# nikhilTkur/Multigrid_dolfinx

Hardware: AMD Instinct MI355X
Metric: V-cycles/sec + achieved HBM GB/s, 3D Poisson P1 1024³ DoF, 1/2/4/8 MI355X (higher is better)
Workload: dtype f64

## Files before the change

### include/mg_hip.h

```cpp
#ifndef MG_HIP_H
#define MG_HIP_H

#include <stddef.h>
#include <stdint.h>

#ifdef __cplusplus
extern "C" {
#endif

typedef struct mg_context* mg_handle;

enum mg_vec {
    MG_VEC_V = 0,
    MG_VEC_F = 1,
    MG_VEC_R = 2,
    MG_VEC_ERR = 3
};

enum mg_restriction {
    MG_RESTRICT_INJECTION = 0,
    MG_RESTRICT_FULL_WEIGHTING = 1,
    MG_RESTRICT_TABLE = 2,
    MG_RESTRICT_P1_TRANSPOSE = 3
};
// ... 142 lines not shown
    MG_PATH_SWEEP1C = 1,
    MG_PATH_PAIR_CLASS = 2,
    MG_PATH_PAIR_PLAIN = 3,
    MG_PATH_KSWEEP = 4,
    MG_PATH_KSWEEP_ESCAPE = 5,
    MG_PATH_KSWEEP_SLAB = 6,
    MG_PATH_BLOCK = 7,
    MG_PATH_K2D = 8,
    MG_PATH_SMALL = 9,
    MG_PATH_MATRIX_FREE = 10,
    MG_PATH_COUNT = 11
};
int mg_smoother_launches(mg_handle h, int level, int path, int64_t* launches, int64_t* sweeps, int64_t* tail_launches);
int mg_reset_smoother_launches(mg_handle h);

int mg_time_kernel(mg_handle h, const char* kernel, int level, int reps, double* avg_ms);
int mg_sync(mg_handle h);
int mg_memory_bytes(mg_handle h, int64_t* bytes);

#ifdef __cplusplus
}
#endif
#endif
```

### multigrid_dolfinx_amd/_capi.py

```python
from __future__ import annotations

import ctypes as C
import os

import numpy as np

_HERE = os.path.dirname(os.path.abspath(__file__))
LIB_PATH = os.path.join(_HERE, "libmg_hip.so")

MG_VEC_V, MG_VEC_F, MG_VEC_R, MG_VEC_ERR = 0, 1, 2, 3
MG_RESTRICT_INJECTION, MG_RESTRICT_FULL_WEIGHTING, MG_RESTRICT_TABLE, MG_RESTRICT_P1_TRANSPOSE = 0, 1, 2, 3
MG_SMOOTH_JACOBI, MG_SMOOTH_RBGS, MG_SMOOTH_MCGS, MG_SMOOTH_CHEBYSHEV = 0, 1, 2, 3
MG_NORM_L2, MG_NORM_MASS = 0, 1
MG_KAPPA_ARITHMETIC, MG_KAPPA_HARMONIC = 0, 1
MG_NODES_INTERIOR, MG_NODES_ALL = 0, 1
MG_BATCH_MAX = 32
MG_BATCH_JACOBI, MG_BATCH_RESIDUAL, MG_BATCH_SPMV = 0, 1, 2
SMOOTHER_PATHS = ("slice", "sweep1c", "pair_class", "pair_plain", "ksweep", "ksweep_escape", "ksweep_slab", "block", "k2d",
                  "small", "matrix_free")

EXCHANGE_FN = C.CFUNCTYPE(C.c_int, C.c_void_p, C.POINTER(C.c_double), C.POINTER(C.c_double),
                          C.POINTER(C.c_double), C.POINTER(C.c_double), C.c_int64)
ALLREDUCE_FN = C.CFUNCTYPE(C.c_int, C.c_void_p, C.POINTER(C.c_double), C.c_int64)
ALLGATHERV_FN = C.CFUNCTYPE(C.c_int, C.c_void_p, C.POINTER(C.c_double), C.c_int64,
# ... 81 lines not shown
    "mg_prepare_cycle": [_H, C.c_int],
    "mg_norm2": [_H, C.c_int, C.c_int, _dp],
    "mg_quadratic_form": [_H, C.c_int, C.c_int, _dp],
    "mg_set_rhs_true": [_H, C.c_int, C.c_void_p],
    "mg_fmg": [_H, C.c_int, C.c_int, C.c_double, C.c_int, C.c_void_p, _ip],
    "mg_set_mass_csr": [_H, C.c_int, C.c_int64, C.c_int64, C.c_void_p, C.c_int, C.c_void_p, C.c_void_p],
    "mg_set_exact": [_H, C.c_int, C.c_void_p],
    "mg_fmg_ex": [_H, C.c_int, C.c_int, C.c_double, C.c_int, C.c_int, C.c_void_p, C.c_void_p, _ip],
    "mg_pcg": [_H, C.c_int, C.c_double, C.c_int, C.c_void_p, _ip],
    "mg_apply_batch": [_H, C.c_int, C.c_int, C.c_int, C.c_void_p, C.c_void_p, C.c_void_p, C.c_void_p],
    "mg_pcg_batch": [_H, C.c_int, C.c_int, C.c_void_p, C.c_void_p, C.c_double, C.c_int, C.c_void_p, C.c_void_p],
    "mg_batch_info": [_H, _ip, _i64p],
    "mg_release_batch": [_H],
    "mg_counters": [_H, _i64p, _i64p, _i64p, _ip],
    "mg_smoother_launches": [_H, C.c_int, C.c_int, _i64p, _i64p, _i64p],
    "mg_reset_smoother_launches": [_H],
    "mg_time_kernel": [_H, C.c_char_p, C.c_int, C.c_int, _dp],
    "mg_sync": [_H],
    "mg_memory_bytes": [_H, _i64p],
}

_lib = None


class MgError(RuntimeError):
    """A non-zero status from libmg_hip.so; the message is mg_last_error()."""


def build_extension():
    import subprocess
# ... 37 lines not shown
```

### multigrid_dolfinx_amd/csrc/mg_capi.hip

```cpp
#include "../../include/mg_hip.h"
#include "mg_csr_check.h"
#include "mg_kernels.hip.h"
#include "mg_direct.hip.h"
#include "mg_jacobi2.hip.h"
#include "mg_jacobik3d.hip.h"
#include "mg_jacobiblk.hip.h"
#include "mg_lattice.hip.h"
#include "mg_diffusion_mf.hip.h"
#include "mg_diffusion_mf_batch.hip.h"
#include "mg_diffusion_adj.hip.h"
#include "mg_diffusion_flux.hip.h"
#include "mg_diffusion_kappa.hip.h"

#include <dlfcn.h>
#include <rccl/rccl.h>

#include <algorithm>
#include <array>
#include <cmath>
#include <cstdio>
#include <cstdlib>
#include <cstring>
#include <initializer_list>
#include <memory>
// ... 134 lines not shown
    bool sdia = false;
    int wu = 0;
    int up[8] = {0, 0, 0, 0, 0, 0, 0, 0};
    int64_t mlead = 0, mslices = 0;
    DevBuf<unsigned char> cls;
    DevBuf<double> ctab;
    int ncls = 0;
    DevBuf<unsigned char> scls;
    DevBuf<int> s_off;
    DevBuf<double> s_val;
    DevBuf<int> s_cnt;
    int nscls = 0;
    DevBuf<int> s_pack;
    int lm_ntop = 0;
    int lm_top[LM_K] = {0, 0, 0, 0, 0, 0, 0, 0};
    int cmain = 0;
    double cm[8] = {0, 0, 0, 0, 0, 0, 0, 0};
    int64_t cls_lead = 0;
    DevBuf<double> dinv;
    bool mf = false;
    DevBuf<double> kappa;
    int faces = MG_FACES_ALL;
    bool diffusion_hierarchy = false;
    bool react = false;
    DevBuf<double> rdiag;
    int robin = 0;
    DVector v, v2, f, err, ftrue;
    DVector sw;
    DVector fcg_x, fcg_p, fcg_q, fcg_b;
    bool cheb_est_ok = false;
// ... 114 lines not shown
    int fuse_k_shape = -1;
    int fuse_k_segments = 0;
    int timing_force_form = -1;
    int64_t fuse_k_slab_min_rows = (int64_t)1 << 20;
    int fuse_k_slab_min_sweeps = 4;
    int64_t fuse_k_min_rows = (int64_t)1 << 24;
    int64_t fuse_k_small_rows = (int64_t)1 << 22;
    int64_t fuse_k5_min_rows = (int64_t)1 << 26;
    int64_t fuse_k4_min_rows = 0;
    int fuse_k_nt_store = 0;
    int fuse_k_min_side = 32;
    int fuse_k_tail = 1;
    int fuse_k_small_tiles = 0;
    int fuse_k_pf = 1;
    int fuse_k_dpp = 1;
    std::vector<const void*> large_lds_kernels;
    int fuse_shape = 1;
    int fuse_wi = 0;
    int fuse_even = 0;
    int march_sweeps = 1;
    int64_t march_min_rows = (int64_t)1 << 22;
    int march_shape = 0;
    int64_t fuse_small_2d_rows = 2048;
    int fuse_small = 1;
    int fuse_2d = 1;
    int fuse_2d_k = 5;
    int fuse_xcd_chunk = 32;
    int cls_blocks_per_cu = 4;
    DirectSolver direct;
    DevTemp ptab_count;
// ... 1217 lines not shown
    MG_TRY(escape_window_k<5>(c, L, cls, clead, &most));
    if (most <= (unsigned)jk3_pool(5)) { *kmax = 5; return 0; }
    MG_TRY(escape_window_k<4>(c, L, cls, clead, &most));
    if (most <= (unsigned)jk3_pool(4)) { *kmax = 4; return 0; }
    MG_TRY(escape_window_k<3>(c, L, cls, clead, &most));
    if (most <= (unsigned)jk3_pool(3)) *kmax = 3;
    return 0;
}

struct JK3Range { int za0, za1, zb0, zb1; };

int jk3_shape(const mg_context* c, int K) {
    return c->fuse_k_shape >= 0 ? c->fuse_k_shape : (K >= 5 ? 8 : 7);
}

template <int K, int NW, int LPW, int M, bool DPP, int PF = 1, int WPE = (NW == 12 ? 3 : 2), int TR = 256, bool ESC = false, bool B1 = false>
int launch_jacobikc_t(mg_context* c, JK3Args a, bool finest, const JK3Range& zr, int seglen) {
    constexpr int EX = 64 * M, EY = NW * LPW, WI = EX - 2 * K, HY = EY - 2 * K + 2;
    a.ntx = (a.nx + WI - 1) / WI;
    a.nty = (a.ny + HY - 1) / HY;
    const int64_t ntile = (int64_t)a.ntx * a.nty;
    constexpr size_t lds = B1 ? jk3b_lds_bytes<K, NW, LPW, M, TR>() : jk3_lds_bytes<K, NW, LPW, M, TR, ESC>();
    static_assert(lds <= 160 * 1024, "one CU's LDS");
    a.za0 = zr.za0; a.za1 = zr.za1; a.zb0 = zr.zb0; a.zb1 = zr.zb1;
    const int planes = std::max(0, zr.za1 - zr.za0) + std::max(0, zr.zb1 - zr.zb0);
    if (planes <= 0) return 0;
    a.ta = (int)ntile; a.seglen_b = 1;
    int64_t items = 0;
    if (seglen <= 0) {
        int64_t cus = std::max(1, c->prop.multiProcessorCount) * (int64_t)std::max<size_t>(1, std::min<size_t>(160 * 1024 / lds, (size_t)(4 * WPE / NW)));
// ... 30 lines not shown
    if (a.ncls > TR) return fail("more row classes than this tile shape keeps in LDS");
    void (*kern)(JK3Args) = nullptr;
    if constexpr (ESC) kern = sdia_jacobikc_escape<K, NW, LPW, M, DPP, PF, WPE, TR>;
    else if constexpr (B1) kern = finest ? sdia_jacobikc_finest_b1<K, NW, LPW, M, WPE, TR> : sdia_jacobikc_b1<K, NW, LPW, M, WPE, TR>;
    else kern = finest ? sdia_jacobikc_finest<K, NW, LPW, M, DPP, PF, WPE, TR> : sdia_jacobikc<K, NW, LPW, M, DPP, PF, WPE, TR>;
    MG_TRY(allow_large_lds(c, reinterpret_cast<const void*>(kern), lds));
    hipLaunchKernelGGL(kern, dim3(grid), dim3(NW * WAVE), lds, c->stream, a);
    HIP_TRY(hipGetLastError());
    c->jk3_tail = a.ta < ntile ? 1 : 0;
    return 0;
}

template <int K, int PF>
int launch_jacobikc_kp(mg_context* c, const JK3Args& a, bool finest, const JK3Range& zr, int seglen) {
    if (!c->fuse_k_dpp) return launch_jacobikc_t<K, 12, 2, 2, false, PF>(c, a, finest, zr, seglen);
    int shape = jk3_shape(c, K) >= 3 && a.ncls > 64 ? 1 : jk3_shape(c, K);
    if (shape == 1 && a.ncls <= 64 && K <= 4 && c->fuse_k_small_tiles) {
        constexpr int WI = 64 - 2 * K, HY = 48 - 2 * K + 2;
        if ((int64_t)((a.nx + WI - 1) / WI) * ((a.ny + HY - 1) / HY) < std::max(1, c->prop.multiProcessorCount)) shape = 4;
    }
    switch (shape) {
        case 1: return launch_jacobikc_t<K, 12, 4, 1, true, PF>(c, a, finest, zr, seglen);
        case 2: return launch_jacobikc_t<K, 8, 3, 2, true, PF>(c, a, finest, zr, seglen);
        case 3: return launch_jacobikc_t<K, 6, 4, 1, true, PF, 3, 64>(c, a, finest, zr, seglen);
        case 4: return launch_jacobikc_t<K, 8, 3, 1, true, PF, 4, 64>(c, a, finest, zr, seglen);
        case 5: if constexpr (K <= 4) return launch_jacobikc_t<K, 4, 6, 1, true, PF, 2, 64>(c, a, finest, zr, seglen);
        case 6: if constexpr (K <= 4 && PF == 1) return launch_jacobikc_t<K, 16, 3, 1, true, 1, 4>(c, a, finest, zr, seglen);
        case 7: return launch_jacobikc_t<K, 16, 2, 1, true, PF, 4>(c, a, finest, zr, seglen);
        case 8: if constexpr (PF == 1) return launch_jacobikc_t<K, 16, 2, 1, true, 1, 4, 256, false, true>(c, a, finest, zr, seglen);
                else return fail("tile shape 8 stages one plane of x (fuse_k_pf 1)");
        default: return launch_jacobikc_t<K, 12, 2, 2, true, PF>(c, a, finest, zr, seglen);
// ... 1 lines not shown
}

template <int K>
int launch_jacobikc_k(mg_context* c, const JK3Args& a, bool finest, const JK3Range& zr, int seglen) {
    if (a.escape) {
        if constexpr (K >= 3) return launch_jacobikc_t<K, 16, 2, 1, true, 1, 4, 256, true>(c, a, finest, zr, seglen);
        else return fail("levels with escape rows take three to five sweeps per pass");
    }
    if constexpr (K == 3 || K == 4) {
        if (c->fuse_k_pf == 2 && (K == 3 || jk3_shape(c, K) == 7)) return launch_jacobikc_kp<K, 2>(c, a, finest, zr, seglen);
    }
    if constexpr (K == 2) return launch_jacobikc_t<K, 12, 4, 1, true, 1>(c, a, finest, zr, seglen);
    else return launch_jacobikc_kp<K, 1>(c, a, finest, zr, seglen);
}

int launch_jacobikc(mg_context* c, const Level& L, int K, const double* x_rows, const double* f_rows, double* out_rows,
                    const JK3Range* zr = nullptr, int seglen = 0) {
    JK3Args a{};
    a.x = x_rows; a.f = f_rows; a.out = out_rows;
    fill_classes_lead(a, L);
    a.P = L.g.plane; a.nx = L.g.nx; a.ny = L.g.ny; a.nz = L.g.nk; a.omega = c->omega;
    const bool dist = is_slab(c, L);
    a.plo = dist && c->comm.rank > 0 ? K : 0;
    a.phi = dist && c->comm.rank + 1 < c->comm.world ? K : 0;
    if (dist && (L.hd < K || L.cls_halo != 1)) return fail("the level's halos are not prepared for that many sweeps per pass");
    if (L.cls_escape && K > L.esc_kmax) return fail("too many escape rows per tile for that many sweeps per pass");
    a.force_form = c->timing_force_form;
    a.nt_store = c->fuse_k_nt_store;
    a.escape = L.cls_escape ? 1 : 0; a.dvals = L.dvals; a.mlead = L.mlead; a.sshift = L.R == 1 ? 6 : (L.R == 2 ? 7 : 8);
    const JK3Range whole{0, L.g.nk, 0, 0};
    c->jk3_tail = 0;
    int rc = 0;
    if (!with_int<2, 3, 4, 5>(K, [&](auto k) { rc = launch_jacobikc_k<decltype(k)::value>(c, a, is_finest(c, L), zr ? *zr : whole, seglen); }))
        return fail("sweeps per pass must be in 2..5");
    return rc;
}

int check_coloring(mg_context* c, Level& L) {
    MG_TRY(need_stored_rows(c, L, "the colouring check of the Gauss-Seidel smoothers"));
    EllArgs a{};
    a.vals = L.vals; a.cols = L.cols; a.codes = L.codes; a.offsets = L.offsets; a.W = L.W;
    a.nloc = L.nloc; a.lead = L.g.lead; a.dinv = L.dinv; a.color_kind = COLOR_LATTICE9; a.grow0 = L.row0; a.gnx = L.g.nx; a.gny = L.g.ny;
    int* d_flag = reinterpret_cast<int*>(c->partials.get());
// ... 1169 lines not shown
                return fail("level " + std::to_string(l) + " is a matrix-free diffusion level: Gauss-Seidel smoothers (RBGS, MCGS) "
                            "need stored rows; use Jacobi or Chebyshev");
    if (!c->direct.tried) { MG_TRY(build_direct(c)); MG_TRY(validate_direct(c)); }
    if (c->smoother == MG_SMOOTH_MCGS)
        for (int l = 1; l <= level; ++l)
            if (c->L[l].mc_ok < 0 && !c->L[l].flat) MG_TRY(check_coloring(c, c->L[l]));
    if (c->comm.active())
        for (int l = 1; l <= level; ++l)
            if (!c->L[l].replicated) {
                MG_TRY(vec_alloc(c, c->L[l], &c->L[l].sw));
                if (c->L[l].cls_halo == 0 && slab_ksweep_level(c, c->L[l]) && std::max(c->mu1, c->mu2) >= c->fuse_k_slab_min_sweeps)
                    MG_TRY(ensure_class_halos(c, c->L[l]));
            }
    if (c->keep_err)
        for (int l = 1; l <= level; ++l) MG_TRY(vec_alloc(c, c->L[l], &c->L[l].err));
    if (c->smoother == MG_SMOOTH_CHEBYSHEV)
        for (int l = 1; l <= level; ++l) {
            double lo = 0.0, hi = 0.0;
            MG_TRY(cheb_interval(c, l, &lo, &hi));
        }
    if (c->p1_prolong || c->restriction == MG_RESTRICT_P1_TRANSPOSE)
        for (int l = 0; l <= level; ++l) MG_TRY(check_p1_stencil(c, c->L[l]));
    return 0;
}

int vcycle_graphed(mg_context* c, int level) {
    MG_TRY(prepare_cycle(c, level));
    const bool slabs = c->comm.active();
    if (!c->use_graph || level == 0 || !c->direct.ok || (slabs && !(c->graph_comm && c->comm.nccl))) return vcycle(c, level);
    std::vector<double*> pre(level + 1);
// ... 626 lines not shown
            return 0;
        }();
        escape = !rc && (double)hist[CLS_ESCAPE] <= 0.25 * (double)L.nloc;
        int kmax = 0;
        if (escape && hist[CLS_ESCAPE] > 0) {
            rc = escape_kmax(c, L, cls, cls_lead, &kmax);
            escape = !rc && kmax >= 3;
        }
        if (std::getenv("MG_DEBUG_STORAGE"))
            std::fprintf(stderr, "[mg] row dictionary with escape: %lld rows, tolerance %d bits, %u escape rows, sweeps per pass that fit %d, rc %d\n",
                         (long long)L.nloc, qbits, hist[CLS_ESCAPE], kmax, rc);
        if (escape) { h[0] = 254; h[1] = 0; L.esc_kmax = kmax; L.rep_escape = hist[CLS_ESCAPE]; }
    }
    if (rc || h[0] > 255 || h[1]) return rc;
    L.cls = std::move(cls); L.ctab = std::move(ctab); L.ncls = h[0] + 1; L.cls_lead = cls_lead;
    L.cls_escape = escape && L.rep_escape > 0;
    if (escape) hist[CLS_ESCAPE] = 0;
    L.cmain = 0;
    for (int k = 1; k < L.ncls; ++k)
        if (L.cmain == 0 || hist[k] > hist[L.cmain]) L.cmain = k;
    for (int t = 0; t < 8; ++t) L.cm[t] = tab[(size_t)CLS_W * L.cmain + t];
    if (L.wu == 4 && !L.cls_escape && !L.flat && L.up[1] == 1 && L.up[2] == L.g.nx && (int64_t)L.up[3] == L.g.plane) {
        JBCheckArgs k{};
        k.cls = L.cls + L.cls_lead; k.ctab = L.ctab; k.nx = L.g.nx; k.ny = L.g.ny; k.nz = L.g.nk; k.P = L.g.plane; k.n = L.nloc;
        k.flag = reinterpret_cast<int*>(c->partials.get());
        HIP_TRY(hipMemsetAsync(k.flag, 0, sizeof(int), c->stream));
        hipLaunchKernelGGL(sdia_grid_decoupled, dim3(blocks_for(L.nloc, 256)), dim3(256), 0, c->stream, k);
        HIP_TRY(hipGetLastError());
        int flag = 1;
        HIP_TRY(hipMemcpyAsync(&flag, k.flag, sizeof(int), hipMemcpyDeviceToHost, c->stream));
// ... 683 lines not shown
    } else if (k == "fuse_k_nt_store") {
        c->fuse_k_nt_store = value != 0;
    } else if (k == "fuse_k_min_side") {
        if (value < 16 || value > 32) return fail("fuse_k_min_side must be in 16..32");
        c->fuse_k_min_side = (int)value;
    } else if (k == "fuse_k_tail") {
        if (value < 0) return fail("fuse_k_tail must be >= 0");
        c->fuse_k_tail = (int)value;
    } else if (k == "fuse_k_small_tiles") {
        c->fuse_k_small_tiles = value != 0;
    } else if (k == "fuse_k_pf") {
        if (value != 1 && value != 2) return fail("fuse_k_pf must be 1 or 2");
        c->fuse_k_pf = (int)value;
    } else if (k == "fuse_k_dpp") {
        c->fuse_k_dpp = value != 0;
    } else if (k == "fuse_k_segments") {
        if (value < 0) return fail("fuse_k_segments must be >= 0");
        c->fuse_k_segments = (int)value;
    } else if (k == "fuse_classes") {
        c->fuse_classes = value != 0;
    } else if (k == "fuse_nontemporal") {
        c->fuse_nontemporal = value != 0;
    } else if (k == "fuse_segments") {
        if (value < 0) return fail("fuse_segments must be >= 0");
        c->fuse_segments = (int)value;
    } else if (k == "coarse_direct") {
        c->use_direct = value != 0;
        free_direct(c);
    } else if (k == "pcg_chunk") {
        if (value < 1) return fail("pcg_chunk must be positive");
// ... 1368 lines not shown
    if (!c) return fail("null handle");
    if (uploads) *uploads = c->uploads;
    if (downloads) *downloads = c->downloads;
    if (graph_replays) *graph_replays = c->graph_replays;
    if (graphs_cached) *graphs_cached = (int)c->graphs.size();
    return 0;
}

int mg_smoother_launches(mg_handle c, int level, int path, int64_t* launches, int64_t* sweeps, int64_t* tail_launches) {
    MG_TRY(check_level(c, level, false));
    if (path < 0 || path >= MG_PATH_COUNT) return fail("smoother path " + std::to_string(path) + " out of range");
    const auto& n = c->smoother_counts[(size_t)level][(size_t)path];
    if (launches) *launches = n.launches;
    if (sweeps) *sweeps = n.sweeps;
    if (tail_launches) *tail_launches = n.tail;
    return 0;
}

int mg_reset_smoother_launches(mg_handle c) {
    if (!c) return fail("null handle");
    for (auto& level : c->smoother_counts) level.fill({});
    return 0;
}

int mg_prepare_cycle(mg_handle c, int level) {
    MG_TRY(check_level(c, level));
    for (int l = 0; l <= level; ++l) {
        MG_TRY(need_matrix(c, l));
        if (level > 0) MG_TRY(need_grid(c, l));
    }
// ... 403 lines not shown
```

### multigrid_dolfinx_amd/csrc/mg_jacobik3d.hip.h

```cpp
#pragma once
#include "mg_jacobi2.hip.h"
#include <type_traits>

namespace mgk {

struct JK3Args {
    const double* x;
    const double* f;
    double* out;
    const unsigned char* cls;
    const double* ctab;
    int64_t clead, P;
    int ncls, cmain;
    double cm[8];
    double omega;
    int nx, ny, nz;
    int plo, phi;
    int ntx, nty, seglen, za0, za1, zb0, zb1;
    int ta, seglen_b;
    unsigned nitems, xcd_chunk;
    int nt_store;
    int escape;
    const double* dvals;
    int64_t mlead;
    int sshift;
    int force_form;
};

constexpr int jk3_pool(int K) { return K >= 5 ? 512 : 1024; }

template <int K, int NW, int LPW, int M, int TR> constexpr size_t jk3_lds_doubles() {
    return TR * CLS_W + (size_t)K * (NW * LPW + 2) * (64 * M) + 2 * (64 * M + 2);
}
template <int K, int NW, int LPW, int M, int TR> constexpr size_t jk3b_lds_doubles() {
    return TR * CLS_W + (size_t)(2 * (K - 1) * (NW * LPW + 1) + 1) * (64 * M);
}
template <int K, int NW, int LPW, int M, int TR> constexpr size_t jk3b_lds_bytes() {
    return sizeof(double) * jk3b_lds_doubles<K, NW, LPW, M, TR>();
}

template <int K, int NW, int LPW, int M, int TR, bool ESC = false> constexpr size_t jk3_lds_bytes() {
    constexpr size_t base = jk3_lds_doubles<K, NW, LPW, M, TR>();
// ... 133 lines not shown
        fn(caps_all{});
    };
    auto cap_of = [&](int c) -> int {
        if constexpr (!CAPS) return K;
        const int ey = ey0 + c / M;
        int cap = min(min(ey + 1, EY - ey), K);
        asm volatile("" : "+v"(cap));
        return __builtin_amdgcn_readfirstlane(cap);
    };

    const int bias = 2 * a.nx + K + 2;
    const int xcl = a.nx + 1 - tx0;
    unsigned eo[NC], eor[M];
#pragma unroll
    for (int c = 0; c < NC; ++c)
        eo[c] = 8u * (unsigned)(min(max(ty0 + ey0 + c / M, -2), a.ny + 1) * a.nx + tx0 + min(lane + 64 * (c % M), xcl) + bias);
#pragma unroll
    for (int r = 0; r < M; ++r)
        eor[r] = 8u * (unsigned)((wlo ? max(ty0 - 1, -2) : min(ty0 + EY, a.ny + 1)) * a.nx + tx0 + min(lane + 64 * r, xcl) + bias);
    unsigned eos[B1 ? M : 1], eon[B1 ? M : 1];
    if constexpr (B1) {
#pragma unroll
        for (int r = 0; r < M; ++r) {
            eos[r] = 8u * (unsigned)(min(max(ty0 + ey0 - 1, -2), a.ny + 1) * a.nx + tx0 + min(lane + 64 * r, xcl) + bias);
            eon[r] = 8u * (unsigned)(min(max(ty0 + ey0 + LPW, -2), a.ny + 1) * a.nx + tx0 + min(lane + 64 * r, xcl) + bias);
        }
    }
    const unsigned char* const clsb = a.cls + a.clead - bias;
    const double* const xb0 = a.x - bias;
    const double* const fb0 = a.f - bias;
    auto sbase = [](const void* p) -> gcptr_t {
        const unsigned long long u = (unsigned long long)p;
        const unsigned lo = (unsigned)__builtin_amdgcn_readfirstlane((int)(unsigned)u);
        const unsigned hi = (unsigned)__builtin_amdgcn_readfirstlane((int)(unsigned)(u >> 32));
        return (gcptr_t)(((unsigned long long)hi << 32) | lo);
    };
    auto ldd = [](gcptr_t b, unsigned e8) -> double {
        asm volatile("" : "+v"(e8));
        return *(const __attribute__((address_space(1))) double*)(b + e8);
    };
    typedef unsigned int __attribute__((aligned(1))) u32_unaligned_t;
    auto ldc = [](gcptr_t b, unsigned e8) -> int {
        unsigned e = e8 >> 3;
        asm volatile("" : "+v"(e));
        return (int)*(const __attribute__((address_space(1))) u32_unaligned_t*)(b + e);
    };
    const int pmin = -a.plo - 1, pmax = a.nz + a.phi;

    double acc[K][NC], fr[K][NC];
    double XA[NC], XB[PF == 2 ? NC : 1], hyA[M], hyB[PF == 2 ? M : 1];
    int CA[NC], CB[PF == 2 ? NC : 1];
    double FN[PF == 2 ? NC : 1];
    unsigned cw[K + 1][CW];
    unsigned long long fast = 0;
    constexpr unsigned long long ALLFAST = (NC * (K + 1) == 64) ? ~0ull : ((1ull << (NC * (K + 1))) - 1ull);
#pragma unroll
    for (int c = 0; c < NC; ++c) {
#pragma unroll
        for (int t = 0; t < K; ++t) acc[t][c] = fr[t][c] = 0.0;
        XA[c] = 0.0;
        CA[c] = 0;
    }
#pragma unroll
    for (int j = 0; j <= K; ++j)
#pragma unroll
        for (int q = 0; q < CW; ++q) cw[j][q] = 0u;
#pragma unroll
    for (int r = 0; r < M; ++r) hyA[r] = hS[r] = hN[r] = 0.0;
    XB[0] = 0.0; hyB[0] = 0.0; CB[0] = 0; FN[0] = 0.0;
#pragma unroll
    for (int c = 0; c < (B1 ? NC : 1); ++c) XP[c] = 0.0;

    auto load_slice = [&](const int i, const int n, const int plane, const int fplane, double (&X)[NC], int (&C)[NC], double (&hy)[M])
        __attribute__((always_inline)) {
        const int64_t o = (int64_t)min(max(plane, pmin), pmax) * a.P;
        const gcptr_t cb = sbase(clsb + o);
        const gcptr_t xb = sbase(xb0 + o);
        const gcptr_t fb = sbase(fb0 + (int64_t)min(max(fplane, pmin), pmax) * a.P);
#pragma unroll
        for (int c = 0; c < NC; ++c) {
            if ((c * n) / NC != i) continue;
            X[c] = ldd(xb, eo[c]);
            C[c] = ldc(cb, eo[c]);
            if constexpr (PF == 2) FN[c] = ldd(fb, eo[c]);
            else fr[K - 1][c] = ldd(fb, eo[c]);
        }
        if constexpr (B1) {
            if (i == n - 1) {
#pragma unroll
                for (int r = 0; r < M; ++r) { hS[r] = ldd(xb, eos[r]); hN[r] = ldd(xb, eon[r]); }
            }
        } else if (i == n - 1 && (wlo || whi)) {
#pragma unroll
            for (int r = 0; r < M; ++r) hy[r] = ldd(xb, eor[r]);
        }
    };
    auto cls_of = [&](int j, int c) -> int { return (int)((cw[j][c / CPR] >> (CBITS * (c % CPR))) & CMASK); };
    auto cls_now = [&](int j, int c) -> int {
// ... 193 lines not shown
                    int (&CN)[PF == 2 ? NC : 1], double (&hyN)[PF == 2 ? M : 1]) __attribute__((always_inline)) {
        k_plane = k; k_store = k >= z0;
        if constexpr (B1) {
            bcur = TR * CLS_W + ey0 * EX + lane + (k & 1) * PS;
            bprev = TR * CLS_W + ey0 * EX + lane + ((k + 1) & 1) * PS;
            asm volatile("" : "+v"(bcur));
            asm volatile("" : "+v"(bprev));
        }
        {
            const unsigned long long u = (unsigned long long)(a.out - bias + (int64_t)k * a.P);
            const unsigned lo = (unsigned)__builtin_amdgcn_readfirstlane((int)(unsigned)u);
            const unsigned hi = (unsigned)__builtin_amdgcn_readfirstlane((int)(unsigned)(u >> 32));
            k_out = (__attribute__((address_space(1))) char*)(((unsigned long long)hi << 32) | lo);
        }
#pragma unroll
        for (int c = 0; c < NC; ++c) {
            asm volatile("" : "+v"(C[c]));
            asm volatile("" : "+v"(X[c]));
            C[c] &= 255;
        }
        if constexpr (ESC) {
            if (a.escape) {
                const int64_t mp = (int64_t)min(max(k + K, pmin), pmax) * a.P - bias + a.mlead;
                const int sh = a.sshift;
                const double* const dv = a.dvals;
                auto at = [&](int64_t m, int slot) -> double { return dv[((((m >> sh) << 2) + slot) << sh) + (m & (((int64_t)1 << sh) - 1))]; };
                unsigned long long em[NC];
                unsigned total = 0u;
#pragma unroll
                for (int c = 0; c < NC; ++c) {
                    if (C[c] == CLS_ESCAPE && (standin >> c & 1u)) C[c] = 0;
                    em[c] = __ballot(C[c] == CLS_ESCAPE);
                    total += (unsigned)__popcll(em[c]);
                }
                if (total != 0u) {
                    unsigned b0 = 0u;
                    if (lane == 0) b0 = atomicAdd(esc_count, total);
                    b0 = (unsigned)__builtin_amdgcn_readfirstlane((int)b0);
                    double e[NC][7];
#pragma unroll
                    for (int c = 0; c < NC; ++c) {
                        if (C[c] == CLS_ESCAPE) {
                            const int64_t m = mp + (int64_t)(eo[c] >> 3);
                            e[c][0] = at(m - a.P, 3); e[c][1] = at(m - a.nx, 2); e[c][2] = at(m - 1, 1);
                            e[c][3] = at(m, 0); e[c][4] = at(m, 1); e[c][5] = at(m, 2); e[c][6] = at(m, 3);
                        }
                    }
#pragma unroll
                    for (int c = 0; c < NC; ++c) {
                        if (C[c] == CLS_ESCAPE) {
                            const unsigned below = __builtin_amdgcn_mbcnt_hi((unsigned)(em[c] >> 32), __builtin_amdgcn_mbcnt_lo((unsigned)em[c], 0u));
                            const int row = DYN0 + (int)((b0 + below) & (unsigned)(jk3_pool(K) - 1));
                            double* const tr = sT + CLS_W * row;
#pragma unroll
                            for (int i = 0; i < 7; ++i) tr[i] = e[c][i];
                            tr[7] = a.omega * (1.0 / (e[c][3] != 0.0 ? e[c][3] : 1.0));
                            C[c] = row;
                        }
                        b0 += (unsigned)__popcll(em[c]);
                    }
                }
            }
        }
        {
            unsigned m = 0;
#pragma unroll
            for (int q = 0; q < CW; ++q) cw[K][q] = 0u;
#pragma unroll
            for (int c = 0; c < NC; ++c) {
                cw[K][c / CPR] |= (unsigned)C[c] << (CBITS * (c % CPR));
                if (__builtin_amdgcn_readfirstlane((int)(__ballot(C[c] != cmain) == 0ull))) m |= 1u << c;
            }
            fast |= (unsigned long long)m << (K * NC);
        }
        int form = 2;
        if ((a.plo > 0 || k >= 1) && (a.phi > 0 || k + K + 1 < a.nz)) {
            if (fast == ALLFAST) {
                form = 0;
            } else {
                bool same = true;
#pragma unroll
                for (int j = 0; j <= K; ++j)
#pragma unroll
                    for (int c = 0; c < NC; ++c) same = same && cls_of(j, c) == cls_of(0, c);
                if (__builtin_amdgcn_readfirstlane((int)(__ballot(!same) == 0ull))) form = 1;
            }
        }
        if (a.force_form >= 0) form = a.force_form;
        if constexpr (CAPS) {
            if (form == 0) by_caps([&](auto caps) __attribute__((always_inline)) { phase_a_fast(std::false_type{}, caps, X); });
            else if (form == 1) by_caps([&](auto caps) __attribute__((always_inline)) { phase_a_fast(std::true_type{}, caps, X); });
            else phase_a_general(X);
        } else {
            if (form == 0) phase_a_fast(std::false_type{}, caps_all{}, X);
            else if (form == 1) phase_a_fast(std::true_type{}, caps_all{}, X);
            else phase_a_general(X);
        }
        if constexpr (B1) {
#pragma unroll
            for (int c = 0; c < NC; ++c) XP[c] = X[c];
        } else if (wlo || whi) {
            double* const ring = image(0) + (wlo ? -EX : LPW * EX);
#pragma unroll
            for (int r = 0; r < M; ++r) ring[64 * r] = hy[r];
        }
#pragma unroll
        for (int c = 0; c < NC; ++c) {
#pragma unroll
            for (int j = 0; j + 1 < K; ++j) fr[j][c] = fr[j + 1][c];
            asm volatile("" : "+v"(fr[K - 2][c]));
        }
#pragma unroll
        for (int j = 0; j < K; ++j)
#pragma unroll
            for (int q = 0; q < CW; ++q) cw[j][q] = cw[j + 1][q];
        fast >>= NC;
        __syncthreads();
        if constexpr (PF == 2) {
#pragma unroll
            for (int c = 0; c < NC; ++c) {
                X[c] = XN[c]; C[c] = CN[c]; fr[K - 1][c] = FN[c];
                asm volatile("" : "+v"(X[c]));
                asm volatile("" : "+v"(C[c]));
                asm volatile("" : "+v"(fr[K - 1][c]));
            }
            if (wlo || whi) {
#pragma unroll
                for (int r = 0; r < M; ++r) { hy[r] = hyN[r]; asm volatile("" : "+v"(hy[r])); }
            }
        }
        auto issue = [&](const int i, const int n) __attribute__((always_inline)) {
            __builtin_amdgcn_sched_barrier(0);
            if constexpr (PF == 2) load_slice(i, n, k + K + 2, k + K + 1, XN, CN, hyN);
            else load_slice(i, n, k + K + 1, k + K, X, C, hy);
            __builtin_amdgcn_sched_barrier(0);
        };
#pragma unroll
        for (int t = 1; t <= K; ++t) {
            if constexpr (CAPS) {
                if (form == 0) by_caps([&](auto caps) __attribute__((always_inline)) { phase_b_fast(std::false_type{}, caps, t, X); });
                else if (form == 1) by_caps([&](auto caps) __attribute__((always_inline)) { phase_b_fast(std::true_type{}, caps, t, X); });
                else phase_b_general(t, X);
            } else {
                if (form == 0) phase_b_fast(std::false_type{}, caps_all{}, t, X);
                else if (form == 1) phase_b_fast(std::true_type{}, caps_all{}, t, X);
                else phase_b_general(t, X);
            }
            issue(t - 1, K);
        }
        if constexpr (!B1) __syncthreads();
    };

    load_slice(0, 1, z0 - K, z0 - K - 1, XA, CA, hyA);
    if constexpr (PF == 2) {
#pragma unroll
        for (int c = 0; c < NC; ++c) fr[K - 1][c] = FN[c];
        load_slice(0, 1, z0 - K + 1, z0 - K, XB, CB, hyB);
    }
    __syncthreads();

    for (int k = z0 - 2 * K; k < z1; ++k) step(k, XA, CA, hyA, XB, CB, hyB);
}

template <int K, int NW, int LPW, int M, bool DPP, int PF, int WPE, int TR>
__global__ __attribute__((amdgpu_flat_work_group_size(NW * WAVE, NW * WAVE), amdgpu_waves_per_eu(WPE, WPE)))
void sdia_jacobikc(JK3Args a) {
    jk3_body<K, NW, LPW, M, DPP, PF, TR>(a);
}

template <int K, int NW, int LPW, int M, bool DPP, int PF, int WPE, int TR>
__global__ __attribute__((amdgpu_flat_work_group_size(NW * WAVE, NW * WAVE), amdgpu_waves_per_eu(WPE, WPE)))
void sdia_jacobikc_finest(JK3Args a) {
// ... 40 lines not shown
            if (ex > xcl || line < -2 || line > a.ny + 1) continue;
            const int64_t row = (int64_t)p * a.P + (int64_t)line * a.nx + tx0 + ex;
            n += a.cls[a.clead + row] == CLS_ESCAPE ? 1u : 0u;
        }
        if (n) atomicAdd(&s_plane, n);
        __syncthreads();
        if (threadIdx.x == 0) {
            win += s_plane - (p >= W ? s_ring[p % W] : 0u);
            s_ring[p % W] = s_plane;
            best = max(best, win);
        }
    }
    if (threadIdx.x == 0 && best) atomicMax(a.most, best);
}

}
```

### multigrid_dolfinx_amd/hierarchy.py

```python
from __future__ import annotations

import ctypes as C
from typing import Dict, Optional

import numpy as np
import scipy.sparse as sp

from . import _capi
from ._capi import (MG_RESTRICT_FULL_WEIGHTING, MG_RESTRICT_INJECTION, MG_VEC_ERR, MG_VEC_F, MG_VEC_R,
                    MG_VEC_V, check, load, ptr)
from . import poisson
from .poisson import face_set, grid_index_from_coords

__all__ = ["DeviceHierarchy", "jacobi_split", "csr_check"]

CHEB_LOWER_RATIO = 6.0

_VEC = {"v": MG_VEC_V, "f": MG_VEC_F, "r": MG_VEC_R, "err": MG_VEC_ERR}
_RESTRICT = {"direct": MG_RESTRICT_INJECTION, "injection": MG_RESTRICT_INJECTION,
             "full_weighting": MG_RESTRICT_FULL_WEIGHTING, "table": _capi.MG_RESTRICT_TABLE,
             "p1_transpose": _capi.MG_RESTRICT_P1_TRANSPOSE}
_NODE_SETS = {"interior": _capi.MG_NODES_INTERIOR, "all": _capi.MG_NODES_ALL}


# ... 765 lines not shown
        return {"uploads": int(up.value), "downloads": int(down.value), "graph_replays": int(rep.value),
                "graphs_cached": int(cached.value)}

    def smoother_launches(self, level: int) -> dict:
        out = {}
        for i, name in enumerate(_capi.SMOOTHER_PATHS):
            n, s, t = C.c_int64(), C.c_int64(), C.c_int64()
            check(self._lib.mg_smoother_launches(self._h, self._idx(level), i, C.byref(n), C.byref(s), C.byref(t)))
            if n.value or s.value or t.value:
                out[name] = (int(n.value), int(s.value), int(t.value))
        return out

    def reset_smoother_launches(self):
        check(self._lib.mg_reset_smoother_launches(self._h))

    def set_level_grid(self, level: int, grid_index=None):
        n = self.n_dofs(level)
        gi = None
        if grid_index is not None:
            gi = np.ascontiguousarray(grid_index, dtype=np.int64)
            if gi.size != n:
                raise ValueError("grid_index has the wrong length")
            if np.array_equal(gi, np.arange(n)):
                gi = None
        check(self._lib.mg_set_level_grid(self._h, self._idx(level), self.elements(level), n,
                                          ptr(gi) if gi is not None else None))

    def set_flat_level(self, A, prune_zeros: bool = True):
        indptr, is64, indices, data = _csr_arrays(A)
        check(self._lib.mg_set_level_csr(self._h, 0, 0, A.shape[0], data.size, ptr(indptr), is64, ptr(indices),
# ... 11 lines not shown
```

Baseline: 4.468.

## Precompute per-wave z-ranges of uniform row classes to skip class loads in Jacobi march

Adds a setup kernel that scans the row-class array for each tile wave. For every wave it records the longest run of z-planes where all classes equal the main class, and the longest run where classes stay constant. The fused K-sweep Jacobi kernel reads this plan and, inside that range, skips the per-plane class byte loads, the ballots and the form selection. This removes class-map traffic and divergent bookkeeping from the inner march, at the cost of a one-time plan build with a host sync and extra branch logic that may raise register pressure.

```diff
diff --git a/include/mg_hip.h b/include/mg_hip.h
--- a/include/mg_hip.h
+++ b/include/mg_hip.h
@@ -180,6 +180,8 @@
 int mg_smoother_launches(mg_handle h, int level, int path, int64_t* launches, int64_t* sweeps, int64_t* tail_launches);
 int mg_reset_smoother_launches(mg_handle h);
 
+int mg_march_plan(mg_handle h, int level, int sweeps, int64_t* waves, int64_t* planes, int64_t* const_waves, int64_t* const_planes);
+
 int mg_time_kernel(mg_handle h, const char* kernel, int level, int reps, double* avg_ms);
 int mg_sync(mg_handle h);
 int mg_memory_bytes(mg_handle h, int64_t* bytes);
diff --git a/multigrid_dolfinx_amd/_capi.py b/multigrid_dolfinx_amd/_capi.py
--- a/multigrid_dolfinx_amd/_capi.py
+++ b/multigrid_dolfinx_amd/_capi.py
@@ -119,6 +119,7 @@
     "mg_release_batch": [_H],
     "mg_counters": [_H, _i64p, _i64p, _i64p, _ip],
     "mg_smoother_launches": [_H, C.c_int, C.c_int, _i64p, _i64p, _i64p],
+    "mg_march_plan": [_H, C.c_int, C.c_int, _i64p, _i64p, _i64p, _i64p],
     "mg_reset_smoother_launches": [_H],
     "mg_time_kernel": [_H, C.c_char_p, C.c_int, C.c_int, _dp],
     "mg_sync": [_H],
diff --git a/multigrid_dolfinx_amd/csrc/mg_capi.hip b/multigrid_dolfinx_amd/csrc/mg_capi.hip
--- a/multigrid_dolfinx_amd/csrc/mg_capi.hip
+++ b/multigrid_dolfinx_amd/csrc/mg_capi.hip
@@ -172,6 +172,11 @@
     DevBuf<int> s_pack;
     int lm_ntop = 0;
     int lm_top[LM_K] = {0, 0, 0, 0, 0, 0, 0, 0};
+    struct MarchPlan {
+        DevBuf<int> iv;
+        int64_t waves[2] = {0, 0}, planes[2] = {0, 0};
+    };
+    MarchPlan plan[6];
     int cmain = 0;
     double cm[8] = {0, 0, 0, 0, 0, 0, 0, 0};
     int64_t cls_lead = 0;
@@ -316,6 +321,7 @@
     int fuse_k_small_tiles = 0;
     int fuse_k_pf = 1;
     int fuse_k_dpp = 1;
+    int fuse_k_plan = 1;
     std::vector<const void*> large_lds_kernels;
     int fuse_shape = 1;
     int fuse_wi = 0;
@@ -1563,6 +1569,40 @@
     return c->fuse_k_shape >= 0 ? c->fuse_k_shape : (K >= 5 ? 8 : 7);
 }
 
+int jk3_shape_for(const mg_context* c, int K, int ncls) {
+    return jk3_shape(c, K) >= 3 && ncls > 64 ? 1 : jk3_shape(c, K);
+}
+
+int march_plan_slot(const mg_context* c, const Level& L, int K) {
+    if (!c->fuse_k_plan || !c->fuse_k_dpp || K < 3 || K > 5 || !L.cls || L.cls_escape || is_slab(c, L)) return -1;
+    const int shape = jk3_shape_for(c, K, L.ncls);
+    return shape == 7 || shape == 8 ? (K - 3) * 2 + (shape - 7) : -1;
+}
+
+int ensure_march_plan(mg_context* c, Level& L, int K, int slot) {
+    Level::MarchPlan& mp = L.plan[slot];
+    if (mp.iv) return 0;
+    JK3PlanArgs a{};
+    a.cls = L.cls; a.clead = L.cls_lead; a.P = L.g.plane; a.nx = L.g.nx; a.ny = L.g.ny; a.nz = L.g.nk; a.cmain = L.cmain;
+    const int WI = 64 - 2 * K, HY = 32 - 2 * K + 2;
+    a.ntx = (a.nx + WI - 1) / WI; a.nty = (a.ny + HY - 1) / HY;
+    const size_t n = (size_t)a.ntx * a.nty * 16 * 4;
+    DevBuf<int> iv;
+    MG_TRY(iv.alloc(c, n));
+    a.plan = iv;
+    with_int<3, 4, 5>(K, [&](auto k) { hipLaunchKernelGGL((jk3_plan<decltype(k)::value, 16, 2, 1>), dim3((unsigned)(a.ntx * a.nty)), dim3(16 * WAVE), 0, c->stream, a); });
+    HIP_TRY(hipGetLastError());
+    std::vector<int> h(n);
+    HIP_TRY(hipMemcpyAsync(h.data(), iv, n * sizeof(int), hipMemcpyDeviceToHost, c->stream));
+    HIP_TRY(hipStreamSynchronize(c->stream));
+    for (size_t i = 0; i < n; i += 4) {
+        if (h[i + 1] > h[i]) { ++mp.waves[0]; mp.planes[0] += h[i + 1] - h[i]; }
+        if (h[i + 3] > h[i + 2] && (h[i + 2] != h[i] || h[i + 3] != h[i + 1])) { ++mp.waves[1]; mp.planes[1] += h[i + 3] - h[i + 2]; }
+    }
+    mp.iv = std::move(iv);
+    return 0;
+}
+
 template <int K, int NW, int LPW, int M, bool DPP, int PF = 1, int WPE = (NW == 12 ? 3 : 2), int TR = 256, bool ESC = false, bool B1 = false>
 int launch_jacobikc_t(mg_context* c, JK3Args a, bool finest, const JK3Range& zr, int seglen) {
     constexpr int EX = 64 * M, EY = NW * LPW, WI = EX - 2 * K, HY = EY - 2 * K + 2;
@@ -1623,7 +1663,7 @@
 template <int K, int PF>
 int launch_jacobikc_kp(mg_context* c, const JK3Args& a, bool finest, const JK3Range& zr, int seglen) {
     if (!c->fuse_k_dpp) return launch_jacobikc_t<K, 12, 2, 2, false, PF>(c, a, finest, zr, seglen);
-    int shape = jk3_shape(c, K) >= 3 && a.ncls > 64 ? 1 : jk3_shape(c, K);
+    int shape = jk3_shape_for(c, K, a.ncls);
     if (shape == 1 && a.ncls <= 64 && K <= 4 && c->fuse_k_small_tiles) {
         constexpr int WI = 64 - 2 * K, HY = 48 - 2 * K + 2;
         if ((int64_t)((a.nx + WI - 1) / WI) * ((a.ny + HY - 1) / HY) < std::max(1, c->prop.multiProcessorCount)) shape = 4;
@@ -1655,7 +1695,7 @@
     else return launch_jacobikc_kp<K, 1>(c, a, finest, zr, seglen);
 }
 
-int launch_jacobikc(mg_context* c, const Level& L, int K, const double* x_rows, const double* f_rows, double* out_rows,
+int launch_jacobikc(mg_context* c, Level& L, int K, const double* x_rows, const double* f_rows, double* out_rows,
                     const JK3Range* zr = nullptr, int seglen = 0) {
     JK3Args a{};
     a.x = x_rows; a.f = f_rows; a.out = out_rows;
@@ -1668,6 +1708,14 @@
     if (L.cls_escape && K > L.esc_kmax) return fail("too many escape rows per tile for that many sweeps per pass");
     a.force_form = c->timing_force_form;
     a.nt_store = c->fuse_k_nt_store;
+    if (const int slot = march_plan_slot(c, L, K); slot >= 0 && a.force_form < 0 && !zr) {
+        if (!L.plan[slot].iv) {
+            hipStreamCaptureStatus st = hipStreamCaptureStatusNone;
+            HIP_TRY(hipStreamIsCapturing(c->stream, &st));
+            if (st == hipStreamCaptureStatusNone) MG_TRY(ensure_march_plan(c, L, K, slot));
+        }
+        a.plan = L.plan[slot].iv;
+    }
     a.escape = L.cls_escape ? 1 : 0; a.dvals = L.dvals; a.mlead = L.mlead; a.sshift = L.R == 1 ? 6 : (L.R == 2 ? 7 : 8);
     const JK3Range whole{0, L.g.nk, 0, 0};
     c->jk3_tail = 0;
@@ -2867,6 +2915,14 @@
             }
     if (c->keep_err)
         for (int l = 1; l <= level; ++l) MG_TRY(vec_alloc(c, c->L[l], &c->L[l].err));
+    if (c->smoother == MG_SMOOTH_JACOBI)
+        for (int l = 1; l <= level; ++l) {
+            Level& L = c->L[l];
+            if (L.mf || is_slab(c, L) || !sweepsk_ok(c, L)) continue;
+            for (const int mu : {c->mu1, c->mu2})
+                for (int nw = mu, k; nw >= 3 && (k = next_pass(nw, sweepsk_max(c, L))) >= 3; nw -= k)
+                    if (const int slot = march_plan_slot(c, L, k); slot >= 0) MG_TRY(ensure_march_plan(c, L, k, slot));
+        }
     if (c->smoother == MG_SMOOTH_CHEBYSHEV)
         for (int l = 1; l <= level; ++l) {
             double lo = 0.0, hi = 0.0;
@@ -3523,6 +3579,7 @@
     }
     if (rc || h[0] > 255 || h[1]) return rc;
     L.cls = std::move(cls); L.ctab = std::move(ctab); L.ncls = h[0] + 1; L.cls_lead = cls_lead;
+    for (auto& mp : L.plan) mp = Level::MarchPlan{};
     L.cls_escape = escape && L.rep_escape > 0;
     if (escape) hist[CLS_ESCAPE] = 0;
     L.cmain = 0;
@@ -4236,6 +4293,8 @@
         c->fuse_k_pf = (int)value;
     } else if (k == "fuse_k_dpp") {
         c->fuse_k_dpp = value != 0;
+    } else if (k == "fuse_k_plan") {
+        c->fuse_k_plan = value != 0;
     } else if (k == "fuse_k_segments") {
         if (value < 0) return fail("fuse_k_segments must be >= 0");
         c->fuse_k_segments = (int)value;
@@ -5634,6 +5693,22 @@
     if (launches) *launches = n.launches;
     if (sweeps) *sweeps = n.sweeps;
     if (tail_launches) *tail_launches = n.tail;
+    return 0;
+}
+
+int mg_march_plan(mg_handle c, int level, int sweeps, int64_t* waves, int64_t* planes, int64_t* const_waves, int64_t* const_planes) {
+    MG_TRY(check_level(c, level));
+    const Level& L = c->L[level];
+    int64_t* const out[4] = {waves, planes, const_waves, const_planes};
+    for (int64_t* o : out)
+        if (o) *o = 0;
+    const int slot = march_plan_slot(c, L, sweeps);
+    if (slot < 0 || !L.plan[slot].iv) return 0;
+    const Level::MarchPlan& mp = L.plan[slot];
+    if (waves) *waves = mp.waves[0];
+    if (planes) *planes = mp.planes[0];
+    if (const_waves) *const_waves = mp.waves[1];
+    if (const_planes) *const_planes = mp.planes[1];
     return 0;
 }
 
diff --git a/multigrid_dolfinx_amd/csrc/mg_jacobik3d.hip.h b/multigrid_dolfinx_amd/csrc/mg_jacobik3d.hip.h
--- a/multigrid_dolfinx_amd/csrc/mg_jacobik3d.hip.h
+++ b/multigrid_dolfinx_amd/csrc/mg_jacobik3d.hip.h
@@ -25,7 +25,15 @@
     int64_t mlead;
     int sshift;
     int force_form;
+    const int* plan;
 };
+
+__device__ __forceinline__ unsigned jk3_cell_offset(int line, int col, int nx, int ny, int tx0, int xcl, int bias) {
+    return 8u * (unsigned)(min(max(line, -2), ny + 1) * nx + tx0 + min(col, xcl) + bias);
+}
+__device__ __forceinline__ const unsigned char* jk3_class_base(const unsigned char* cls, int64_t clead, int bias) {
+    return cls + clead - bias;
+}
 
 constexpr int jk3_pool(int K) { return K >= 5 ? 512 : 1024; }
 
@@ -189,7 +197,7 @@
     unsigned eo[NC], eor[M];
 #pragma unroll
     for (int c = 0; c < NC; ++c)
-        eo[c] = 8u * (unsigned)(min(max(ty0 + ey0 + c / M, -2), a.ny + 1) * a.nx + tx0 + min(lane + 64 * (c % M), xcl) + bias);
+        eo[c] = jk3_cell_offset(ty0 + ey0 + c / M, lane + 64 * (c % M), a.nx, a.ny, tx0, xcl, bias);
 #pragma unroll
     for (int r = 0; r < M; ++r)
         eor[r] = 8u * (unsigned)((wlo ? max(ty0 - 1, -2) : min(ty0 + EY, a.ny + 1)) * a.nx + tx0 + min(lane + 64 * r, xcl) + bias);
@@ -197,11 +205,11 @@
     if constexpr (B1) {
 #pragma unroll
         for (int r = 0; r < M; ++r) {
-            eos[r] = 8u * (unsigned)(min(max(ty0 + ey0 - 1, -2), a.ny + 1) * a.nx + tx0 + min(lane + 64 * r, xcl) + bias);
-            eon[r] = 8u * (unsigned)(min(max(ty0 + ey0 + LPW, -2), a.ny + 1) * a.nx + tx0 + min(lane + 64 * r, xcl) + bias);
-        }
-    }
-    const unsigned char* const clsb = a.cls + a.clead - bias;
+            eos[r] = jk3_cell_offset(ty0 + ey0 - 1, lane + 64 * r, a.nx, a.ny, tx0, xcl, bias);
+            eon[r] = jk3_cell_offset(ty0 + ey0 + LPW, lane + 64 * r, a.nx, a.ny, tx0, xcl, bias);
+        }
+    }
+    const unsigned char* const clsb = jk3_class_base(a.cls, a.clead, bias);
     const double* const xb0 = a.x - bias;
     const double* const fb0 = a.f - bias;
     auto sbase = [](const void* p) -> gcptr_t {
@@ -222,6 +230,27 @@
     };
     const int pmin = -a.plo - 1, pmax = a.nz + a.phi;
 
+    constexpr bool PLANNED = !ESC && NW == 16 && LPW == 2 && M == 1 && K >= 3;
+    int klo = 0x7fffffff, khi = 0x7fffffff, kform = 0;
+    if constexpr (PLANNED) {
+        if (a.plan) {
+            const int* const pw = a.plan + 4 * ((int)tt * NW + wave);
+            const int top = a.nz - K - 1;
+            const int lo0 = max(max(pw[0], 1), z0 - K), hi0 = min(pw[1] - K, top);
+            const int lo1 = max(max(pw[2], 1), z0 - K), hi1 = min(pw[3] - K, top);
+            const int n0 = min(hi0, z1) - lo0, n1 = min(hi1, z1) - lo1;
+            if (n0 > 0 && n0 >= n1) {
+                klo = __builtin_amdgcn_readfirstlane(lo0);
+                khi = __builtin_amdgcn_readfirstlane(hi0);
+            } else if (n1 > 0) {
+                klo = __builtin_amdgcn_readfirstlane(lo1);
+                khi = __builtin_amdgcn_readfirstlane(hi1);
+                kform = 1;
+            }
+        }
+    }
+    auto interior_step = [&](int k) -> bool { return PLANNED && k >= klo && k < khi; };
+
     double acc[K][NC], fr[K][NC];
     double XA[NC], XB[PF == 2 ? NC : 1], hyA[M], hyB[PF == 2 ? M : 1];
     int CA[NC], CB[PF == 2 ? NC : 1];
@@ -246,7 +275,7 @@
 #pragma unroll
     for (int c = 0; c < (B1 ? NC : 1); ++c) XP[c] = 0.0;
 
-    auto load_slice = [&](const int i, const int n, const int plane, const int fplane, double (&X)[NC], int (&C)[NC], double (&hy)[M])
+    auto load_slice = [&](const int i, const int n, const int plane, const int fplane, const bool noc, double (&X)[NC], int (&C)[NC], double (&hy)[M])
         __attribute__((always_inline)) {
         const int64_t o = (int64_t)min(max(plane, pmin), pmax) * a.P;
         const gcptr_t cb = sbase(clsb + o);
@@ -256,7 +285,7 @@
         for (int c = 0; c < NC; ++c) {
             if ((c * n) / NC != i) continue;
             X[c] = ldd(xb, eo[c]);
-            C[c] = ldc(cb, eo[c]);
+            if (!noc) C[c] = ldc(cb, eo[c]);
             if constexpr (PF == 2) FN[c] = ldd(fb, eo[c]);
             else fr[K - 1][c] = ldd(fb, eo[c]);
         }
@@ -480,76 +509,96 @@
             k_out = (__attribute__((address_space(1))) char*)(((unsigned long long)hi << 32) | lo);
         }
 #pragma unroll
-        for (int c = 0; c < NC; ++c) {
-            asm volatile("" : "+v"(C[c]));
-            asm volatile("" : "+v"(X[c]));
-            C[c] &= 255;
-        }
-        if constexpr (ESC) {
-            if (a.escape) {
-                const int64_t mp = (int64_t)min(max(k + K, pmin), pmax) * a.P - bias + a.mlead;
-                const int sh = a.sshift;
-                const double* const dv = a.dvals;
-                auto at = [&](int64_t m, int slot) -> double { return dv[((((m >> sh) << 2) + slot) << sh) + (m & (((int64_t)1 << sh) - 1))]; };
-                unsigned long long em[NC];
-                unsigned total = 0u;
-#pragma unroll
-                for (int c = 0; c < NC; ++c) {
-                    if (C[c] == CLS_ESCAPE && (standin >> c & 1u)) C[c] = 0;
-                    em[c] = __ballot(C[c] == CLS_ESCAPE);
-                    total += (unsigned)__popcll(em[c]);
-                }
-                if (total != 0u) {
-                    unsigned b0 = 0u;
-                    if (lane == 0) b0 = atomicAdd(esc_count, total);
-                    b0 = (unsigned)__builtin_amdgcn_readfirstlane((int)b0);
-                    double e[NC][7];
+        for (int c = 0; c < NC; ++c) asm volatile("" : "+v"(X[c]));
+        const bool interior = interior_step(k);
+        if constexpr (PLANNED) {
+            if (k == khi) {
+                unsigned m = 0;
+#pragma unroll
+                for (int c = 0; c < NC; ++c)
+                    if (__builtin_amdgcn_readfirstlane((int)(__ballot(cls_of(0, c) != cmain) == 0ull))) m |= 1u << c;
+                fast = 0;
+#pragma unroll
+                for (int j = 0; j < K; ++j) {
+                    fast |= (unsigned long long)m << (j * NC);
+#pragma unroll
+                    for (int q = 0; q < CW; ++q) cw[j][q] = cw[0][q];
+                }
+            }
+        }
+        int form = kform;
+        if (!interior) {
+#pragma unroll
+            for (int c = 0; c < NC; ++c) {
+                asm volatile("" : "+v"(C[c]));
+                C[c] &= 255;
+            }
+            if constexpr (ESC) {
+                if (a.escape) {
+                    const int64_t mp = (int64_t)min(max(k + K, pmin), pmax) * a.P - bias + a.mlead;
+                    const int sh = a.sshift;
+                    const double* const dv = a.dvals;
+                    auto at = [&](int64_t m, int slot) -> double { return dv[((((m >> sh) << 2) + slot) << sh) + (m & (((int64_t)1 << sh) - 1))]; };
+                    unsigned long long em[NC];
+                    unsigned total = 0u;
 #pragma unroll
                     for (int c = 0; c < NC; ++c) {
-                        if (C[c] == CLS_ESCAPE) {
-                            const int64_t m = mp + (int64_t)(eo[c] >> 3);
-                            e[c][0] = at(m - a.P, 3); e[c][1] = at(m - a.nx, 2); e[c][2] = at(m - 1, 1);
-                            e[c][3] = at(m, 0); e[c][4] = at(m, 1); e[c][5] = at(m, 2); e[c][6] = at(m, 3);
+                        if (C[c] == CLS_ESCAPE && (standin >> c & 1u)) C[c] = 0;
+                        em[c] = __ballot(C[c] == CLS_ESCAPE);
+                        total += (unsigned)__popcll(em[c]);
+                    }
+                    if (total != 0u) {
+                        unsigned b0 = 0u;
+                        if (lane == 0) b0 = atomicAdd(esc_count, total);
+                        b0 = (unsigned)__builtin_amdgcn_readfirstlane((int)b0);
+                        double e[NC][7];
+#pragma unroll
+                        for (int c = 0; c < NC; ++c) {
+                            if (C[c] == CLS_ESCAPE) {
+                                const int64_t m = mp + (int64_t)(eo[c] >> 3);
+                                e[c][0] = at(m - a.P, 3); e[c][1] = at(m - a.nx, 2); e[c][2] = at(m - 1, 1);
+                                e[c][3] = at(m, 0); e[c][4] = at(m, 1); e[c][5] = at(m, 2); e[c][6] = at(m, 3);
+                            }
+                        }
+#pragma unroll
+                        for (int c = 0; c < NC; ++c) {
+                            if (C[c] == CLS_ESCAPE) {
+                                const unsigned below = __builtin_amdgcn_mbcnt_hi((unsigned)(em[c] >> 32), __builtin_amdgcn_mbcnt_lo((unsigned)em[c], 0u));
+                                const int row = DYN0 + (int)((b0 + below) & (unsigned)(jk3_pool(K) - 1));
+                                double* const tr = sT + CLS_W * row;
+#pragma unroll
+                                for (int i = 0; i < 7; ++i) tr[i] = e[c][i];
+                                tr[7] = a.omega * (1.0 / (e[c][3] != 0.0 ? e[c][3] : 1.0));
+                                C[c] = row;
+                            }
+                            b0 += (unsigned)__popcll(em[c]);
                         }
                     }
-#pragma unroll
-                    for (int c = 0; c < NC; ++c) {
-                        if (C[c] == CLS_ESCAPE) {
-                            const unsigned below = __builtin_amdgcn_mbcnt_hi((unsigned)(em[c] >> 32), __builtin_amdgcn_mbcnt_lo((unsigned)em[c], 0u));
-                            const int row = DYN0 + (int)((b0 + below) & (unsigned)(jk3_pool(K) - 1));
-                            double* const tr = sT + CLS_W * row;
-#pragma unroll
-                            for (int i = 0; i < 7; ++i) tr[i] = e[c][i];
-                            tr[7] = a.omega * (1.0 / (e[c][3] != 0.0 ? e[c][3] : 1.0));
-                            C[c] = row;
-                        }
-                        b0 += (unsigned)__popcll(em[c]);
-                    }
-                }
-            }
-        }
-        {
-            unsigned m = 0;
-#pragma unroll
-            for (int q = 0; q < CW; ++q) cw[K][q] = 0u;
-#pragma unroll
-            for (int c = 0; c < NC; ++c) {
-                cw[K][c / CPR] |= (unsigned)C[c] << (CBITS * (c % CPR));
-                if (__builtin_amdgcn_readfirstlane((int)(__ballot(C[c] != cmain) == 0ull))) m |= 1u << c;
-            }
-            fast |= (unsigned long long)m << (K * NC);
-        }
-        int form = 2;
-        if ((a.plo > 0 || k >= 1) && (a.phi > 0 || k + K + 1 < a.nz)) {
-            if (fast == ALLFAST) {
-                form = 0;
-            } else {
-                bool same = true;
-#pragma unroll
-                for (int j = 0; j <= K; ++j)
-#pragma unroll
-                    for (int c = 0; c < NC; ++c) same = same && cls_of(j, c) == cls_of(0, c);
-                if (__builtin_amdgcn_readfirstlane((int)(__ballot(!same) == 0ull))) form = 1;
+                }
+            }
+            {
+                unsigned m = 0;
+#pragma unroll
+                for (int q = 0; q < CW; ++q) cw[K][q] = 0u;
+#pragma unroll
+                for (int c = 0; c < NC; ++c) {
+                    cw[K][c / CPR] |= (unsigned)C[c] << (CBITS * (c % CPR));
+                    if (__builtin_amdgcn_readfirstlane((int)(__ballot(C[c] != cmain) == 0ull))) m |= 1u << c;
+                }
+                fast |= (unsigned long long)m << (K * NC);
+            }
+            form = 2;
+            if ((a.plo > 0 || k >= 1) && (a.phi > 0 || k + K + 1 < a.nz)) {
+                if (fast == ALLFAST) {
+                    form = 0;
+                } else {
+                    bool same = true;
+#pragma unroll
+                    for (int j = 0; j <= K; ++j)
+#pragma unroll
+                        for (int c = 0; c < NC; ++c) same = same && cls_of(j, c) == cls_of(0, c);
+                    if (__builtin_amdgcn_readfirstlane((int)(__ballot(!same) == 0ull))) form = 1;
+                }
             }
         }
         if (a.force_form >= 0) form = a.force_form;
@@ -576,11 +625,13 @@
             for (int j = 0; j + 1 < K; ++j) fr[j][c] = fr[j + 1][c];
             asm volatile("" : "+v"(fr[K - 2][c]));
         }
-#pragma unroll
-        for (int j = 0; j < K; ++j)
-#pragma unroll
-            for (int q = 0; q < CW; ++q) cw[j][q] = cw[j + 1][q];
-        fast >>= NC;
+        if (!interior) {
+#pragma unroll
+            for (int j = 0; j < K; ++j)
+#pragma unroll
+                for (int q = 0; q < CW; ++q) cw[j][q] = cw[j + 1][q];
+            fast >>= NC;
+        }
         __syncthreads();
         if constexpr (PF == 2) {
 #pragma unroll
@@ -597,8 +648,8 @@
         }
         auto issue = [&](const int i, const int n) __attribute__((always_inline)) {
             __builtin_amdgcn_sched_barrier(0);
-            if constexpr (PF == 2) load_slice(i, n, k + K + 2, k + K + 1, XN, CN, hyN);
-            else load_slice(i, n, k + K + 1, k + K, X, C, hy);
+            if constexpr (PF == 2) load_slice(i, n, k + K + 2, k + K + 1, interior_step(k + 2), XN, CN, hyN);
+            else load_slice(i, n, k + K + 1, k + K, interior_step(k + 1), X, C, hy);
             __builtin_amdgcn_sched_barrier(0);
         };
 #pragma unroll
@@ -617,11 +668,11 @@
         if constexpr (!B1) __syncthreads();
     };
 
-    load_slice(0, 1, z0 - K, z0 - K - 1, XA, CA, hyA);
+    load_slice(0, 1, z0 - K, z0 - K - 1, false, XA, CA, hyA);
     if constexpr (PF == 2) {
 #pragma unroll
         for (int c = 0; c < NC; ++c) fr[K - 1][c] = FN[c];
-        load_slice(0, 1, z0 - K + 1, z0 - K, XB, CB, hyB);
+        load_slice(0, 1, z0 - K + 1, z0 - K, false, XB, CB, hyB);
     }
     __syncthreads();
 
@@ -692,4 +743,67 @@
     if (threadIdx.x == 0 && best) atomicMax(a.most, best);
 }
 
-}
+struct JK3PlanArgs {
+    const unsigned char* cls;
+    int64_t clead, P;
+    int nx, ny, nz, ntx, nty, cmain;
+    int* plan;
+};
+
+template <int K, int NW, int LPW, int M>
+__global__ __launch_bounds__(NW * WAVE) void jk3_plan(JK3PlanArgs a) {
+    constexpr int EX = 64 * M, EY = NW * LPW, NC = M * LPW, WI = EX - 2 * K, HY = EY - 2 * K + 2;
+    constexpr int U = 4;
+    const int lane = threadIdx.x & 63;
+    const int wave = __builtin_amdgcn_readfirstlane((int)(threadIdx.x >> 6));
+    const unsigned tt = blockIdx.x;
+    const int tiy = (int)(tt / (unsigned)a.ntx), tix = (int)(tt % (unsigned)a.ntx);
+    const int tx0 = tix * WI - K, ty0 = tiy * HY - (K - 1);
+    const int ey0 = wave * LPW, bias = 2 * a.nx + K + 2, xcl = a.nx + 1 - tx0;
+    unsigned eo[NC];
+#pragma unroll
+    for (int c = 0; c < NC; ++c) eo[c] = jk3_cell_offset(ty0 + ey0 + c / M, lane + 64 * (c % M), a.nx, a.ny, tx0, xcl, bias);
+    const unsigned char* const clsb = jk3_class_base(a.cls, a.clead, bias);
+    int p0 = 0, p1 = 0, prun = 0;
+    int q0 = 0, q1 = 0, qrun = 0;
+    int prev[NC];
+#pragma unroll
+    for (int c = 0; c < NC; ++c) prev[c] = -1;
+    for (int pb = 0; pb < a.nz; pb += U) {
+        int cl[U][NC];
+#pragma unroll
+        for (int u = 0; u < U; ++u) {
+            const unsigned char* const cb = clsb + (int64_t)min(pb + u, a.nz - 1) * a.P;
+#pragma unroll
+            for (int c = 0; c < NC; ++c) cl[u][c] = cb[eo[c] >> 3];
+        }
+#pragma unroll
+        for (int u = 0; u < U; ++u) {
+            const int p = pb + u;
+            if (p >= a.nz) break;
+            bool all = true, same = true;
+#pragma unroll
+            for (int c = 0; c < NC; ++c) {
+                all = all && cl[u][c] == a.cmain;
+                same = same && cl[u][c] == prev[c];
+                prev[c] = cl[u][c];
+            }
+            if (__ballot(!all) != 0ull) {
+                if (p - prun > p1 - p0) { p0 = prun; p1 = p; }
+                prun = p + 1;
+            }
+            if (__ballot(!same) != 0ull) {
+                if (p - qrun > q1 - q0) { q0 = qrun; q1 = p; }
+                qrun = p;
+            }
+        }
+    }
+    if (a.nz - prun > p1 - p0) { p0 = prun; p1 = a.nz; }
+    if (a.nz - qrun > q1 - q0) { q0 = qrun; q1 = a.nz; }
+    if (lane == 0) {
+        int* const pw = a.plan + 4 * ((int)tt * NW + wave);
+        pw[0] = p0; pw[1] = p1; pw[2] = q0; pw[3] = q1;
+    }
+}
+
+}
diff --git a/multigrid_dolfinx_amd/hierarchy.py b/multigrid_dolfinx_amd/hierarchy.py
--- a/multigrid_dolfinx_amd/hierarchy.py
+++ b/multigrid_dolfinx_amd/hierarchy.py
@@ -803,6 +803,11 @@
     def reset_smoother_launches(self):
         check(self._lib.mg_reset_smoother_launches(self._h))
 
+    def march_plan(self, level: int, sweeps: int) -> tuple:
+        out = [C.c_int64() for _ in range(4)]
+        check(self._lib.mg_march_plan(self._h, self._idx(level), sweeps, *[C.byref(v) for v in out]))
+        return tuple(int(v.value) for v in out)
+
     def set_level_grid(self, level: int, grid_index=None):
         n = self.n_dofs(level)
         gi = None
```

Result: faster. 4.798 (median of 6 runs) (+7.4%).
